# florasion/D-VQVAE

Hardware: AMD Instinct MI355X
Metric: grasps/sec at batch=65536, N=1024 pts, K=512 (higher is better)
Workload: dtype f32 (GEMMs: every fp32 operand as two fp16 pieces, a1 = fp16(a), a2 = fp16((a - a1) * 2^11), weights pre-scaled by one power of two per output row; the 3 partial products a1 b1, a1 b2, a2 b1 are exact in fp32 and accumulate in TWO fp32 accumulators (large / cross terms) on v_mfma_f32_16x16x32_f16; d

## Files before the change

### d-vqvae_amd/csrc/pn_filter.h

```cpp
#pragma once
#include <stddef.h>
#include "pn_slots.h"

constexpr int PN_MAX_TILES = 64;
constexpr int PN_MAX_POINTS = PN_MAX_TILES * PN_TILE_SLOTS;

struct PnGeometry {
    int tiles;
    int deal;
    int Npad;
    long slots;
    size_t h2;
    size_t rec4;
    size_t rec2;
    size_t tstat;
    size_t cbuf;
    bool has_tail() const { return deal < tiles; }
    size_t part() const { return rec4 + rec2; }
    size_t per_sample() const { return h2 + part() + tstat + cbuf; }
};
inline PnGeometry pn_geometry(int N, bool tail_enabled) {
    PnGeometry g;
    g.tiles = (N + PN_TILE_SLOTS - 1) / PN_TILE_SLOTS;
    const int over = N - PN_TILE_SLOTS * (g.tiles - 1);
// ... 12 lines not shown
    auto up = [](size_t n) { return (n + 255) / 256 * 256; };
    const size_t part = up(samples * g.h2), tstat = part + up(samples * g.part()), cbuf = tstat + up(samples * g.tstat);
    return {0, part, part + samples * g.rec4, tstat, cbuf, cbuf + up(samples * g.cbuf)};
}

enum PnAbl : int {
    PN_ABL_NO_H2_STORE = 1,
    PN_ABL_NO_CONV3 = 2,
    PN_ABL_FEW_ROWS = 16,
    PN_ABL_NO_GROUPS = 32,
    PN_ABL_NO_DOTS = 64,
    PN_ABL_NO_CHAIN = 128,
    PN_ABL_NO_PUBLISH = 256,
    PN_ABL_NO_HANDOVER = 512,
    PN_ABL_NO_W3_LOADS = 1024,
    PN_ABL_STAMPS = 4096,
    PN_ABL_CLOCK = 8192,
    PN_ABL_NO_CHUNK_BARRIER = 16384,
    PN_ABL_INJECT_LIE = 32768,
    PN_ABL_INJECT_LOST = 65536,
    PN_ABL_CONSUMER = 131072,
    PN_ABL_SPLIT = 262144,
    PN_ABL_ONE_PER_CU = 524288,
    PN_ABL_VALID = PN_ABL_STAMPS | PN_ABL_CLOCK | PN_ABL_INJECT_LIE | PN_ABL_INJECT_LOST | PN_ABL_ONE_PER_CU
};

struct PnSlot { float *h2, *part, *cbuf; void* part2; unsigned* tstat; };

#ifdef __HIPCC__
#include "dvq_internal.h"

struct PnTrunkWeights {
    const float *w1, *b1, *w2, *b2, *w3, *b3;
    const uint16_t *w2p, *w3p;
    const void* w3f;
    int relu3;
};
inline PnTrunkWeights pn_stn_trunk(const dvq_pointnet_weights* w) {
    return {w->s_w1, w->s_b1, w->s_w2, w->s_b2, w->s_w3, w->s_b3, w->s_w2p, w->s_w3p, w->s_w3f, 1};
}
inline PnTrunkWeights pn_main_trunk(const dvq_pointnet_weights* w) {
    return {w->w1, w->b1, w->w2, w->b2, w->w3, w->b3, w->w2p, w->w3p, w->w3f, 0};
}
struct PnBatch { const float *pc, *trans; int C, N; long B; };

int dvq_launch_pn_trunk(const PnBatch& in, const PnTrunkWeights& w, float* partial, hipStream_t st);
int dvq_launch_pn_filter_front(const PnBatch& in, const PnTrunkWeights& w, const PnSlot& sl, unsigned long long* stats, hipStream_t st);
int dvq_launch_pn_filter_back(const PnBatch& in, const PnTrunkWeights& w, const PnSlot& sl, float* feat, long ld_feat,
// ... 6 lines not shown
```

### d-vqvae_amd/csrc/pointnet.hip

```cpp
#include "dvq_internal.h"
#include "pn_filter.h"
#include <map>
#include <utility>
#include <vector>

namespace {

__global__ void pn_layer1_kernel(const float* __restrict__ pc, int C, int N, int Npad, long B,
                                 const float* __restrict__ trans , const float* __restrict__ W ,
                                 const float* __restrict__ bias, float* __restrict__ out ) {
    const long gid = (long)blockIdx.x * blockDim.x + threadIdx.x;
    const long pt = gid >> 4;
    const int q = (int)(gid & 15);
    if (pt >= B * Npad) return;
    const long b = pt / Npad;
    const int n = (int)(pt % Npad);
    f32x4 y = {0.f, 0.f, 0.f, 0.f};
    if (n < N) {
        const float* src = pc + b * (long)C * N;
        float x0 = src[n], x1 = src[N + n], x2 = src[2 * N + n];
        const float x3 = (C > 3) ? src[3 * N + n] : 0.f;
        if (trans) {
            const float* t = trans + b * 9;
            const float n0 = fmaf(x2, t[6], fmaf(x1, t[3], x0 * t[0]));
// ... 33 lines not shown
        const long v = dvq_knobs().pn_chunk;
        if (v > 0 && v < chunk) chunk = v;
        if (v <= 0) {
            if (chunk > 4096) chunk = 4096;
            if (B >= 2048 && chunk > (B + 3) / 4) chunk = (B + 3) / 4;
        }
    }
    if (chunk > B) chunk = B;
    if (chunk < 1) chunk = 1;
    if (B > 0) chunk = (B + ((B + chunk - 1) / chunk) - 1) / ((B + chunk - 1) / chunk);
    s.chunk = chunk;
    const long launches = B > 0 ? (B + chunk - 1) / chunk : 1;
    s.slots = launches >= 2 ? (dvq_knobs().pn_slots > 0 ? dvq_knobs().pn_slots : 2) : 1;
    if (s.slots > 4) s.slots = 4;
    if (s.slots > 2 * launches) s.slots = (int)(2 * launches);
    char* p = (char*)ws;
    auto take = [&](size_t n) { char* q = p; p += dvq_round_up(n, 256); return (float*)q; };
    const PnSetLayout l = pn_set_layout(s.g, (size_t)chunk);
    for (int i = 0; i < s.slots; ++i) {
        char* set = (char*)take(l.bytes);
        s.slot[i] = PnSlot{(float*)(set + l.h2), (float*)(set + l.part), (float*)(set + l.cbuf), set + l.part2, (unsigned*)(set + l.tstat)};
    }
    s.h1 = s.slots >= 2 ? s.slot[1].h2 : take((size_t)chunk * s.g.Npad * 64 * 4);
    s.stats = (unsigned long long*)take(64);
    s.f0 = take((size_t)chunk * 1024 * 4);
    s.f1 = take((size_t)chunk * 512 * 4);
    s.f2 = take((size_t)chunk * 256 * 4);
    s.tr = take((size_t)(B > 0 ? B : 1) * 16 * 4);
    s.bytes = (size_t)(p - (char*)ws);
    return s;
}

int dense(const float* x, int K, const float* w, const uint16_t* wp, const float* b, long M, int N, int relu, float* y, hipStream_t st) {
    GemmParams p = {};
    p.src[0] = GemmSrc{x, w, (long)K, (long)K, K, 0, wp, (long)N * K};
    p.nsrc = 1;
    p.M = M;
    p.N = N;
    p.bias = b;
    p.out = y;
    p.ldo = N;
    p.relu = relu;
    return dvq_launch_gemm(p, EPI_BIAS, st);
}

bool use_filter(const dvq_pointnet_weights* w, int N) {
    const int fm = dvq_knobs().pn_filter;
// ... 385 lines not shown
```

### d-vqvae_amd/csrc/pointnet_filter.hip

```cpp
#include "dvq_internal.h"
#include "pn_filter.h"
#include <vector>

namespace {

typedef __bf16 qbf16x8 __attribute__((ext_vector_type(8)));
typedef _Float16 qf16x8 __attribute__((ext_vector_type(8)));
typedef _Float16 qf16x2 __attribute__((ext_vector_type(2)));
typedef float qf32x2 __attribute__((ext_vector_type(2)));

constexpr float C_ID = 5.0e-5f;
constexpr float DELTA = 1.0e-6f;
constexpr float NEG_BIG = -3.0e38f;

constexpr int F_STAGE2 = 2 * 64 * 128;
constexpr int IMG_OFF_TI = 1024 * 256, IMG_OFF_WN = IMG_OFF_TI + 4096, IMG_OFF_RN = IMG_OFF_WN + 4096;
constexpr int IMG_OFF_W2 = IMG_OFF_RN + 4096, IMG_OFF_K2 = IMG_OFF_W2 + 2 * 128 * 128, IMG_BYTES = IMG_OFF_K2 + 512;
constexpr int F_STAGE3 = 64 * 256;
constexpr int F_OFF_TB = 2 * F_STAGE3;
constexpr int F_SLOT = 4 * 2 * 2 * 2 * 64;
constexpr int F_OFF_W1 = F_OFF_TB + 8 * 4 * 4 * 64 * 4;
constexpr int F_OFF_B1 = F_OFF_W1 + 64 * 4 * 4;
constexpr int F_OFF_B2 = F_OFF_B1 + 64 * 4;
constexpr int F_OFF_K2 = F_OFF_B2 + 128 * 4;
// ... 602 lines not shown
    s = fmaf(w1[0], c[0], s);
    s = fmaf(w1[1], c[1], s);
    s = fmaf(w1[2], c[2], s);
    s = fmaf(w1[3], c[3], s);
    s += q_dpp<0xB1>(s);
    s += q_dpp<0x4E>(s);
    s += q_dpp<0x141>(s);
    s += q_dpp<0x140>(s);
    return s;
}
__device__ __forceinline__ float exact_dot(const f32x4& w0, const f32x4& w1, const float* __restrict__ hrow, int j) {
    return exact_dot_regs(w0, w1, *reinterpret_cast<const f32x4*>(hrow + 4 * j), *reinterpret_cast<const f32x4*>(hrow + 4 * j + 64));
}
__device__ __forceinline__ float max_nan(float a, float b) { return (a != a || b != b) ? __builtin_nanf("") : fmaxf(a, b); }

__device__ __forceinline__ unsigned f2key(float v) {
    const unsigned u = __float_as_uint(v);
    return (u & 0x80000000u) ? ~u : (u | 0x80000000u);
}
__device__ __forceinline__ float key2f(unsigned k) { return __uint_as_float((k & 0x80000000u) ? (k & 0x7fffffffu) : ~k); }

__device__ unsigned long long g_pn_faults[2];

constexpr int PAIR_CAP = 1024;
constexpr int FB_CAP = 512;
constexpr int SORT_CAP = 3072;
__global__ __launch_bounds__(256, 4) void pn_exact_kernel(const f32x4* __restrict__ part, const qf32x2* __restrict__ part2, int tiles, int deal,
                                                       const float* __restrict__ h2buf,
                                                       int N, int Npad, const float* __restrict__ w3, const float* __restrict__ b3,
                                                       const float* __restrict__ wnorm, const float* __restrict__ rnorm,
                                                       const unsigned* __restrict__ tstat, const float* __restrict__ cbuf, int relu, int exhaustive,
                                                       int pair_cap, int fb_cap, float* __restrict__ feat, long ld_feat,
                                                       unsigned long long* __restrict__ stats, int abl_arg) {
    const int abl = DVQ_DIAG_ON ? abl_arg : 0;
    __shared__ unsigned short cand[1024][4];
    __shared__ unsigned char cand_n[1024];
    __shared__ int pair_list[PAIR_CAP];
    __shared__ int fb_list[FB_CAP];
    __shared__ short all_list[1024];
    __shared__ int pair_count, fb_count, all_count;
    __shared__ float fb_part[4][16];
    __shared__ float hm[PN_MAX_TILES], dm[PN_MAX_TILES], rd[PN_MAX_TILES];
    __shared__ unsigned best_k[1024];
    __shared__ int pcnt[1024];
    __shared__ unsigned sorted[SORT_CAP];
    __shared__ int wave_tot[4];
    const int tid = threadIdx.x, g = tid >> 4, j = tid & 15;
    const long b = blockIdx.x;
    float* wcs = reinterpret_cast<float*>(pcnt);
    const f32x4 cen_a = *reinterpret_cast<const f32x4*>(cbuf + b * 128 + 4 * j), cen_b = *reinterpret_cast<const f32x4*>(cbuf + b * 128 + 4 * j + 64);
    if (tid == 0) { pair_count = 0; fb_count = 0; all_count = 0; }
#pragma unroll
    for (int i = 0; i < 4; ++i) pcnt[tid + 256 * i] = 0;
    int nonfinite_point = 0;
    if (tid < tiles) {
        const unsigned* ts = tstat + 4 * (b * tiles + tid);
        hm[tid] = __uint_as_float(ts[0]) * 1.00001f;
        dm[tid] = __uint_as_float(ts[1]) * 1.00001f;
        rd[tid] = __uint_as_float(ts[2]) * 1.00001f;
        nonfinite_point = ts[3] != 0 && !(abl & PN_ABL_STAMPS);
    }
    if (__syncthreads_or(nonfinite_point)) {
        for (int n = tid; n < 1024; n += 256) feat[b * ld_feat + n] = __builtin_nanf("");
        return;
    }
    const float* h2 = h2buf + b * (long)Npad * 128;
    const bool wrap_small = Npad <= 2 * N;
    const f32x4* pt = part + b * (long)tiles * 1024;
    const qf32x2* pt2 = part2 + b * (long)tiles * 1024;
    const bool stamps = DVQ_DIAG_ON && stats && (abl & PN_ABL_STAMPS);
    unsigned long long tp0 = stamps ? __builtin_amdgcn_s_memtime() : 0ull, tp1 = 0, tp2 = 0, tp3 = 0;
    unsigned n_single = 0, n_multi = 0, n_cand = 0, n_wave = 0, n_suspect = 0;
    float lo_0 = 1.f, lo_1 = 1.f, lo_2 = 1.f, lo_3 = 1.f, hi_0 = 0.f, hi_1 = 0.f, hi_2 = 0.f, hi_3 = 0.f;
    f32x4 nf0 = pt[tid], nf1 = pt[min(1, tiles - 1) * 1024 + tid], nf2 = pt[min(2, tiles - 1) * 1024 + tid], nf3 = pt[min(3, tiles - 1) * 1024 + tid];
    qf32x2 ng0 = pt2[tid], ng1 = pt2[min(1, tiles - 1) * 1024 + tid], ng2 = pt2[min(2, tiles - 1) * 1024 + tid], ng3 = pt2[min(3, tiles - 1) * 1024 + tid];
    float nwn = wnorm[tid], nrn = rnorm[tid];
#pragma unroll 1
    for (int ci = 0; ci < 4; ++ci) {
        const int n = tid + 256 * ci;
        best_k[n] = f2key(NEG_BIG);
        const float wn = nwn, rn = nrn;
        const f32x4 f0 = nf0, f1 = nf1, f2 = nf2, f3 = nf3;
        const qf32x2 g0 = ng0, g1 = ng1, g2 = ng2, g3 = ng3;
        if (ci < 3) {
            const int nx = n + 256;
            nf0 = pt[nx]; nf1 = pt[min(1, tiles - 1) * 1024 + nx]; nf2 = pt[min(2, tiles - 1) * 1024 + nx]; nf3 = pt[min(3, tiles - 1) * 1024 + nx];
            ng0 = pt2[nx]; ng1 = pt2[min(1, tiles - 1) * 1024 + nx]; ng2 = pt2[min(2, tiles - 1) * 1024 + nx]; ng3 = pt2[min(3, tiles - 1) * 1024 + nx];
            nwn = wnorm[nx]; nrn = rnorm[nx];
        }
        float lb, e_all;
        auto bound = [&](int t) { return fmaf(rn, dm[t], fmaf(wn, rd[t], fmaf(C_ID * wn, dm[t], 2.0f * DELTA * wn * hm[t]))); };
        bool nonfinite = false;
        float ub;
        auto fold = [&](float e, float top) {
            nonfinite = nonfinite || !(e < 3.0e38f) || !(fabsf(top) < 3.0e38f);
            e_all = fmaxf(e_all, e);
            lb = fmaxf(lb, top - e);
            ub = fmaxf(ub, top + e);
        };
        {
            const float e0 = bound(0);
            e_all = e0;
            lb = f0[0] - e0;
            ub = f0[0] + e0;
            nonfinite = !(e0 < 3.0e38f) || !(fabsf(f0[0]) < 3.0e38f);
            if (tiles > 1) fold(bound(1), f1[0]);
            if (tiles > 2) fold(bound(2), f2[0]);
            if (tiles > 3) fold(bound(3), f3[0]);
        }
        for (int t0 = 4; t0 < tiles; t0 += 4) {
            float top[4];
#pragma unroll
            for (int u = 0; u < 4; ++u) top[u] = pt[min(t0 + u, tiles - 1) * 1024 + n][0];
#pragma unroll
            for (int u = 0; u < 4; ++u)
                if (t0 + u < tiles) fold(bound(t0 + u), top[u]);
        }
        int cands = 0;
        bool whole = false;
        const bool all = exhaustive || nonfinite || !(e_all < 3.0e38f) || !(lb > NEG_BIG) || !(lb < 3.0e38f);
        if (all) {
            all_list[atomicAdd(&all_count, 1)] = (short)n;
            cand_n[n] = 0;
            continue;
        }
        float lo_c = lb, hi_c = ub;
        auto consider = [&](int t, const f32x4& q, const qf32x2& q45) {
            const float et = bound(t);
            const unsigned suspect = (__float_as_uint(q[3]) >> 16) & 1u;
            n_suspect += suspect;
            if (!suspect && !(q[0] + et >= lb)) return;
            unsigned flags = __float_as_uint(q[3]) & 0xFFFFu;
            auto take = [&](float v) {
                int p = point_of_slot(t, slot_of_id(__float_as_uint(v) & 255u), deal);
                if (p >= N) p = wrap_small ? p - N : p % N;
                if (abl & PN_ABL_FEW_ROWS) p &= 63;
                if (cands < 4) cand[n][cands] = (unsigned short)p;
                else {
                    const int slot = atomicAdd(&pair_count, 1);
                    if (slot < pair_cap) pair_list[slot] = n | (p << 10);
                    else {
                        const unsigned id = __float_as_uint(v);
                        flags |= 1u << pn_group_of_id(id);
                    }
                }
                ++cands;
            };
            const float sc5[5] = {q[0], q[1], q[2], q45[0], q45[1]};
#pragma unroll 1
            for (int k = 0; k < 5; ++k) {
                const float v = k == 0 ? sc5[0] : k == 1 ? sc5[1] : k == 2 ? sc5[2] : k == 3 ? sc5[3] : sc5[4];
                if (!(v + et >= lb)) break;
                take(v);
            }
            while (flags) {
                const int wh = __ffs(flags) - 1;
                flags &= flags - 1;
                const int slot = atomicAdd(&fb_count, 1);
                if (slot < fb_cap) fb_list[slot] = n | (t << 10) | (wh << 20);
                else if (!whole) {
                    whole = true;
                    all_list[atomicAdd(&all_count, 1)] = (short)n;
                }
                ++n_wave;
            }
        };
        f32x4 q0 = f0, q1 = f1, q2 = f2, q3 = f3;
        qf32x2 h0 = g0, h1 = g1, h2q = g2, h3 = g3;
#pragma unroll 1
        for (int t0 = 0; t0 < tiles; t0 += 4) {
            if (t0 > 0) {
                q0 = pt[min(t0, tiles - 1) * 1024 + n]; q1 = pt[min(t0 + 1, tiles - 1) * 1024 + n];
                q2 = pt[min(t0 + 2, tiles - 1) * 1024 + n]; q3 = pt[min(t0 + 3, tiles - 1) * 1024 + n];
                h0 = pt2[min(t0, tiles - 1) * 1024 + n]; h1 = pt2[min(t0 + 1, tiles - 1) * 1024 + n];
                h2q = pt2[min(t0 + 2, tiles - 1) * 1024 + n]; h3 = pt2[min(t0 + 3, tiles - 1) * 1024 + n];
            }
#pragma unroll 1
            for (int u = 0; u < 4 && t0 + u < tiles; ++u) {
                const f32x4 q = u == 0 ? q0 : u == 1 ? q1 : u == 2 ? q2 : q3;
                const qf32x2 q45 = u == 0 ? h0 : u == 1 ? h1 : u == 2 ? h2q : h3;
                consider(t0 + u, q, q45);
            }
        }
        cand_n[n] = whole ? 0 : (unsigned char)min(cands, 4);
        if (whole) { lo_c = 1.f; hi_c = 0.f; }
        lo_0 = ci == 0 ? lo_c : lo_0; hi_0 = ci == 0 ? hi_c : hi_0;
        lo_1 = ci == 1 ? lo_c : lo_1; hi_1 = ci == 1 ? hi_c : hi_1;
        lo_2 = ci == 2 ? lo_c : lo_2; hi_2 = ci == 2 ? hi_c : hi_2;
        lo_3 = ci == 3 ? lo_c : lo_3; hi_3 = ci == 3 ? hi_c : hi_3;
        n_single += cands == 1;
        n_multi += cands != 1;
        n_cand += cands;
    }
    dvq_lds_barrier();
    if (stamps) tp1 = __builtin_amdgcn_s_memtime();
    const int npairs = min(pair_count, pair_cap);
    for (int n = tid; n < 1024; n += 256)
        for (int k = 0; k < cand_n[n]; ++k) atomicAdd(&pcnt[cand[n][k] & 1023], 1);
    for (int i = tid; i < npairs; i += 256) atomicAdd(&pcnt[(pair_list[i] >> 10) & 1023], 1);
    dvq_lds_barrier();
    int total;
    {
        const int c0 = pcnt[4 * tid], c1 = pcnt[4 * tid + 1], c2 = pcnt[4 * tid + 2], c3 = pcnt[4 * tid + 3];
        int incl = c0 + c1 + c2 + c3;
#pragma unroll
        for (int o = 1; o < 64; o <<= 1) {
            const int v = __shfl_up(incl, o);
            if ((tid & 63) >= o) incl += v;
        }
        if ((tid & 63) == 63) wave_tot[tid >> 6] = incl;
        dvq_lds_barrier();
        int base = 0;
        for (int w = 0; w < (tid >> 6); ++w) base += wave_tot[w];
        total = wave_tot[0] + wave_tot[1] + wave_tot[2] + wave_tot[3];
        const int excl = base + incl - (c0 + c1 + c2 + c3);
        pcnt[4 * tid] = excl;
        pcnt[4 * tid + 1] = excl + c0;
        pcnt[4 * tid + 2] = excl + c0 + c1;
        pcnt[4 * tid + 3] = excl + c0 + c1 + c2;
    }
    dvq_lds_barrier();
    const bool by_point = total <= SORT_CAP && !(abl & PN_ABL_NO_DOTS);
    if (by_point) {
        for (int n = tid; n < 1024; n += 256)
            for (int k = 0; k < cand_n[n]; ++k) {
                const int p = cand[n][k];
                sorted[atomicAdd(&pcnt[p & 1023], 1)] = (unsigned)n | ((unsigned)p << 10);
            }
        for (int i = tid; i < npairs; i += 256) {
            const int code = pair_list[i];
            sorted[atomicAdd(&pcnt[(code >> 10) & 1023], 1)] = (unsigned)code;
        }
        dvq_lds_barrier();
        if (stamps) tp2 = __builtin_amdgcn_s_memtime();
        const int per = (total + 15) >> 4, i0 = g * per, i1 = min(total, i0 + per);
        for (int i = i0; i < i1; i += 4) {
            f32x4 w0[4], w1[4], ha[4], hb[4];
            int nn[4];
#pragma unroll
            for (int u = 0; u < 4; ++u) {
                const unsigned code = sorted[min(i + u, i1 - 1)];
                nn[u] = (int)(code & 1023u);
                const unsigned woff = (code & 1023u) * 512u + 16u * (unsigned)j, hoff = (code >> 10) * 512u + 16u * (unsigned)j;
                w0[u] = *reinterpret_cast<const f32x4*>(reinterpret_cast<const char*>(w3) + woff);
                w1[u] = *reinterpret_cast<const f32x4*>(reinterpret_cast<const char*>(w3) + woff + 256);
                ha[u] = *reinterpret_cast<const f32x4*>(reinterpret_cast<const char*>(h2) + hoff);
                hb[u] = *reinterpret_cast<const f32x4*>(reinterpret_cast<const char*>(h2) + hoff + 256);
            }
            float v[4], wc[4];
#pragma unroll
            for (int u = 0; u < 4; ++u) {
                v[u] = exact_dot_regs(w0[u], w1[u], ha[u], hb[u]);
                wc[u] = exact_dot_regs(w0[u], w1[u], cen_a, cen_b);
            }
            if (j == 0) {
#pragma unroll
                for (int u = 0; u < 4; ++u)
                    if (i + u < i1) { atomicMax(&best_k[nn[u]], f2key(v[u])); wcs[nn[u]] = wc[u]; }
            }
        }
    }
    for (int n0 = g; n0 < ((abl & PN_ABL_NO_DOTS) || by_point ? 0 : 1024); n0 += 64) {
        f32x4 w0[4], w1[4], ha[4], hb[4];
        int cn[4];
#pragma unroll
        for (int u = 0; u < 4; ++u) {
            const int n = n0 + 16 * u;
            cn[u] = cand_n[n];
            const float* wr = reinterpret_cast<const float*>(reinterpret_cast<const char*>(w3) + ((unsigned)n * 512u + 16u * (unsigned)j));
            w0[u] = *reinterpret_cast<const f32x4*>(wr);
            w1[u] = *reinterpret_cast<const f32x4*>(wr + 64);
            const float* hr = h2 + (long)(cn[u] ? cand[n][0] : 0) * 128 + 4 * j;
            ha[u] = *reinterpret_cast<const f32x4*>(hr);
            hb[u] = *reinterpret_cast<const f32x4*>(hr + 64);
        }
#pragma unroll
        for (int u = 0; u < 4; ++u) {
            const int n = n0 + 16 * u;
            if (cn[u] == 0) continue;
            float best = exact_dot_regs(w0[u], w1[u], ha[u], hb[u]);
            const float wc = exact_dot_regs(w0[u], w1[u], cen_a, cen_b);
            if (j == 0) wcs[n] = wc;
            if (cn[u] > 1) {
                f32x4 xa[3], xb[3];
#pragma unroll
                for (int k = 1; k < 4; ++k)
                    if (k < cn[u]) {
                        const float* hr = h2 + (long)cand[n][k] * 128 + 4 * j;
                        xa[k - 1] = *reinterpret_cast<const f32x4*>(hr);
                        xb[k - 1] = *reinterpret_cast<const f32x4*>(hr + 64);
                    }
#pragma unroll
                for (int k = 1; k < 4; ++k)
                    if (k < cn[u]) best = fmaxf(best, exact_dot_regs(w0[u], w1[u], xa[k - 1], xb[k - 1]));
            }
            if (j == 0) atomicMax(&best_k[n], f2key(best));
        }
    }
    for (int i = g; i < (by_point ? 0 : npairs); i += 16) {
        const int code = pair_list[i];
        const int n = code & 1023;
        const float* wr = reinterpret_cast<const float*>(reinterpret_cast<const char*>(w3) + ((unsigned)n * 512u + 16u * (unsigned)j));
        const float v = exact_dot(*reinterpret_cast<const f32x4*>(wr), *reinterpret_cast<const f32x4*>(wr + 64), h2 + (long)(code >> 10) * 128, j);
        if (j == 0) atomicMax(&best_k[n], f2key(v));
    }
    if (stamps) tp3 = __builtin_amdgcn_s_memtime();
    const int nfb = (abl & PN_ABL_NO_GROUPS) ? 0 : min(fb_count, fb_cap);
    for (int i = tid >> 6; i < nfb; i += 4) {
        const int code = fb_list[i];
        const int n = code & 1023, t = (code >> 10) & 1023, grp = (code >> 20) & 15;
        const float* wr = reinterpret_cast<const float*>(reinterpret_cast<const char*>(w3) + ((unsigned)n * 512u + 16u * (unsigned)j));
        const f32x4 w0 = *reinterpret_cast<const f32x4*>(wr), w1 = *reinterpret_cast<const f32x4*>(wr + 64);
        float best = NEG_BIG;
        {
            f32x4 ha[4], hb[4];
#pragma unroll
            for (int u = 0; u < 4; ++u) {
                int p = point_of_slot(t, pn_group_slot(grp, 4 * (g & 3) + u), deal);
                if (p >= N) p %= N;
                const float* hr = reinterpret_cast<const float*>(reinterpret_cast<const char*>(h2) + ((unsigned)p * 512u + 16u * (unsigned)j));
                ha[u] = *reinterpret_cast<const f32x4*>(hr);
                hb[u] = *reinterpret_cast<const f32x4*>(hr + 64);
            }
#pragma unroll
            for (int u = 0; u < 4; ++u) best = fmaxf(best, exact_dot_regs(w0, w1, ha[u], hb[u]));
        }
        if (j == 0) atomicMax(&best_k[n], f2key(best));
    }
    dvq_lds_barrier();
// ... 36 lines not shown
#pragma unroll
    for (int ci = 0; ci < 4; ++ci) {
        const int n = tid + 256 * ci;
        const float lo_c = ci == 0 ? lo_0 : ci == 1 ? lo_1 : ci == 2 ? lo_2 : lo_3, hi_c = ci == 0 ? hi_0 : ci == 1 ? hi_1 : ci == 2 ? hi_2 : hi_3;
        if (!(lo_c <= hi_c) || (abl & ~PN_ABL_VALID)) continue;
        const float v = key2f(best_k[n]), wc = wcs[n];
        const float x = v - wc, slack = 4.0e-7f * (fabsf(v) + fabsf(wc));
        if (!(x >= lo_c - slack && x <= hi_c + slack)) {
            all_list[atomicAdd(&all_count, 1)] = (short)n;
            ++n_bad;
        }
    }
    dvq_lds_barrier();
    eval_all_list(all_count);
    if (n_suspect) atomicAdd(&g_pn_faults[0], (unsigned long long)n_suspect);
    if (n_bad) atomicAdd(&g_pn_faults[1], (unsigned long long)n_bad);
    for (int n = tid; n < 1024; n += 256) {
        const unsigned k = best_k[n];
        const float v = (k == 0xffffffffu ? __builtin_nanf("") : key2f(k)) + b3[n];
        feat[b * ld_feat + n] = relu ? (v != v ? v : fmaxf(v, 0.f)) : v;
    }
    if (stamps && tid == 0) {
        const unsigned long long t_end = __builtin_amdgcn_s_memtime();
        atomicAdd(stats + 4, tp1 - tp0); atomicAdd(stats + 5, tp2 - tp1); atomicAdd(stats + 6, tp3 - tp2); atomicAdd(stats + 7, t_end - tp3);
    }
    if (stats) {
        if (n_single) atomicAdd(stats + 0, (unsigned long long)n_single);
        if (n_multi) atomicAdd(stats + 1, (unsigned long long)n_multi);
        if (n_wave) atomicAdd(stats + 2, (unsigned long long)n_wave);
        if (n_cand) atomicAdd(stats + 3, (unsigned long long)n_cand);
    }
}

constexpr int CENTER_SPB = 4;
template <int C>
__global__ __launch_bounds__(256) void pn_center_kernel(const float* __restrict__ pc, const float* __restrict__ trans, int N, long B,
                                                        const float* __restrict__ W1, const float* __restrict__ b1,
                                                        const float* __restrict__ W2, const float* __restrict__ b2,
                                                        float* __restrict__ cbuf, unsigned* __restrict__ tstat, int tiles) {
    __shared__ float w2t[64][129];
    __shared__ float h1c[4][64];
    __shared__ float h2c[4][128];
    const int tid = threadIdx.x, q = tid >> 6, k = tid & 63;
    for (int i = tid; i < 128 * 64; i += 256) w2t[i & 63][i >> 6] = W2[i];
    for (int sb = 0; sb < CENTER_SPB; ++sb) {
        const long b = (long)blockIdx.x * CENTER_SPB + sb;
        if (b >= B) break;
        for (int i = tid; i < 4 * tiles; i += 256) tstat[b * 4 * tiles + i] = 0u;
        {
// ... 104 lines not shown
static int pn_abl() { const char* e = getenv("DVQ_PN_ABL"); return e ? atoi(e) : 0; }
#else
static constexpr int pn_abl() { return 0; }
#endif

using TrunkFilterKernel = decltype(&pn_trunk_filter_kernel<3, false>);
static TrunkFilterKernel trunk_filter_kernel(int C, bool tail) {
    static const TrunkFilterKernel k[2][2] = {{&pn_trunk_filter_kernel<3, false>, &pn_trunk_filter_kernel<3, true>},
                                              {&pn_trunk_filter_kernel<4, false>, &pn_trunk_filter_kernel<4, true>}};
    return k[C == 4][tail];
}
static decltype(&pn_center_kernel<3>) center_kernel(int C) { return C == 4 ? &pn_center_kernel<4> : &pn_center_kernel<3>; }

int dvq_launch_pn_filter_front(const PnBatch& in, const PnTrunkWeights& w, const PnSlot& sl, unsigned long long* stats, hipStream_t st) {
    PnGeometry g;
    DVQ_PROPAGATE(filter_geometry(in.N, &g));
    static DvqOncePerDevice attr_once[2][2];
    for (int c = 0; c < 2; ++c)
        for (int tail = 0; tail < 2; ++tail)
            DVQ_PROPAGATE(dvq_lds_limit(attr_once[c][tail], reinterpret_cast<const void*>(trunk_filter_kernel(3 + c, tail)),
                                        tail ? F_LDS_TAIL : (DVQ_DIAG_ON ? 100 * 1024 : F_LDS), "pointnet"));
    const long B = in.B, grid = B * g.deal;
    DVQ_REQUIRE(B * g.tiles < (1L << 31), "pointnet: grid too large");
    if (stats && hipMemsetAsync(stats, 0, 64, st) != hipSuccess) {
        dvq_set_error("pointnet: hipMemsetAsync failed");
        return DVQ_ELAUNCH;
    }
    {
        DVQ_PROF("pn_center", 2.0 * (double)B * 4 * (4.0 * 64 + 64.0 * 128), (double)B * (64 + 512), st);
        DVQ_LAUNCH(center_kernel(in.C), dim3((unsigned)((B + CENTER_SPB - 1) / CENTER_SPB)), dim3(256), 0, st, in.pc, in.trans, in.N, B, w.w1,
                   w.b1, w.w2, w.b2, sl.cbuf, sl.tstat, g.tiles);
    }
    DVQ_CHECK_LAUNCH("pn_center");
    const double pts = (double)B * g.slots;
    const int abl = pn_abl();
    auto launch = [&](bool tail, int lds, hipStream_t s, int abl_arg) {
        DVQ_LAUNCH(trunk_filter_kernel(in.C, tail), dim3((unsigned)(tail ? (B + 3) / 4 : grid)), dim3(256), lds, s, in.pc, in.trans, in.N, g.Npad,
                   g.tiles, g.deal, B, w.w1, w.b1, w.b2, (const char*)w.w3f, sl.h2, (f32x4*)sl.part, (qf32x2*)sl.part2, sl.tstat, sl.cbuf, abl_arg);
    };
    {
        DVQ_PROF("pn_trunk", 2.0 * pts * (4.0 * 64 + 64.0 * 128 + 128.0 * 1024), pts * (16 + 512) + (double)grid * 16384, st);
#ifdef DVQ_DIAG
        if ((abl & PN_ABL_SPLIT) && in.C == 4) {
            static hipStream_t side = nullptr;
            static hipEvent_t ev0 = nullptr, ev1 = nullptr;
            if (!side) { (void)hipStreamCreateWithFlags(&side, hipStreamNonBlocking); (void)hipEventCreateWithFlags(&ev0, hipEventDisableTiming); (void)hipEventCreateWithFlags(&ev1, hipEventDisableTiming); }
            (void)hipEventRecord(ev0, st);
// ... 34 lines not shown
                   reinterpret_cast<const float*>((const char*)w.w3f + IMG_OFF_RN), tstat, sl.cbuf, w.relu3, exhaustive, pair_cap, fb_cap,
                   feat, ld_feat, stats, abl);
    }
    DVQ_CHECK_LAUNCH("pn_exact");
    if (stats && (abl & PN_ABL_STAMPS)) {
        const long nrec = B * tiles;
        std::vector<unsigned> ts((size_t)nrec * 4);
        (void)hipStreamSynchronize(st);
        (void)hipMemcpy(ts.data(), tstat, ts.size() * 4, hipMemcpyDeviceToHost);
        double a = 0, b2_ = 0, c = 0, d = 0;
        for (long i = 0; i < nrec; ++i) {
            const unsigned v = ts[4 * i + 3];
            a += v & 255; b2_ += (v >> 8) & 255; c += (v >> 16) & 255; d += (v >> 24) & 255;
        }
        if (abl & PN_ABL_CLOCK) {
            double mhz = 0;
            for (long i = 0; i < nrec; ++i) mhz += ts[4 * i + 3];
            fprintf(stderr, "[dvq pn] in-kernel clock of the trunk kernel: %.0f MHz (s_memtime over s_memrealtime, mean over %ld workgroups)\n", mhz / nrec, nrec);
        } else
        fprintf(stderr, "[dvq pn] mean phase ticks per workgroup (s_memtime): start->loaded %.0f, conv1+conv2 %.0f, centre/convert %.0f, conv3 loop %.0f\n",
                a / nrec * 64, b2_ / nrec * 64, c / nrec * 64, d / nrec * 512);
    }
    if (stats) {
        unsigned long long h[8] = {0, 0, 0, 0, 0, 0, 0, 0};
        (void)hipStreamSynchronize(st);
        (void)hipMemcpy(h, stats, sizeof h, hipMemcpyDeviceToHost);
        (void)hipMemset((void*)stats, 0, sizeof h);
        const double tot = (double)B * 1024;
        fprintf(stderr, "[dvq pn] B=%ld N=%d: one candidate %.4f, other counts %.4f of the channels, flagged 16-point groups %.5f per channel; %.3f candidate dots per channel\n",
                B, N, h[0] / tot, h[1] / tot, h[2] / tot, h[3] / tot);
        if (abl & PN_ABL_STAMPS)
            fprintf(stderr, "[dvq pn] exact stage, mean cycles per workgroup: records -> candidates %.0f, sort by point %.0f, candidate dots %.0f, flagged groups + checks + store %.0f\n",
                    (double)h[4] / B, (double)h[5] / B, (double)h[6] / B, (double)h[7] / B);
    }
    return DVQ_OK;
}

int dvq_pn_fault_counters(unsigned long long* out2, int reset) {
    if (hipDeviceSynchronize() != hipSuccess || hipMemcpyFromSymbol(out2, HIP_SYMBOL(g_pn_faults), 16) != hipSuccess) {
        dvq_set_error("pointnet_fault_counters: reading the device counters failed");
        return DVQ_ELAUNCH;
    }
    if (reset) {
        const unsigned long long z[2] = {0, 0};
        if (hipMemcpyToSymbol(HIP_SYMBOL(g_pn_faults), z, 16) != hipSuccess) {
            dvq_set_error("pointnet_fault_counters: resetting the device counters failed");
            return DVQ_ELAUNCH;
        }
    }
    return DVQ_OK;
}
```

Baseline: 183,600.

## Add anchor pre-pass with exact dots to tighten candidate pruning in exact stage

The exact max-pool stage now runs a first pass that picks each channel's most likely winning point (anchor), sorts those anchors by point and computes their exact dots up front. The resulting exact value, adjusted by the centre term, raises the lower bound used to prune further candidates (rule 2). A second rule skips flagged 16-point groups whose remaining scores cannot reach the bound (rule 1). The fixed 4-candidate per-channel arrays and the unsorted fallback path are replaced by one sorted pair list with a larger capacity. This trades an extra scan over the tile records and extra barriers for fewer candidate dots and fewer fallback group evaluations.

```diff
diff --git a/d-vqvae_amd/csrc/pn_filter.h b/d-vqvae_amd/csrc/pn_filter.h
--- a/d-vqvae_amd/csrc/pn_filter.h
+++ b/d-vqvae_amd/csrc/pn_filter.h
@@ -58,8 +58,12 @@
     PN_ABL_CONSUMER = 131072,
     PN_ABL_SPLIT = 262144,
     PN_ABL_ONE_PER_CU = 524288,
-    PN_ABL_VALID = PN_ABL_STAMPS | PN_ABL_CLOCK | PN_ABL_INJECT_LIE | PN_ABL_INJECT_LOST | PN_ABL_ONE_PER_CU
+    PN_ABL_NO_RULE1 = 1048576,
+    PN_ABL_NO_RULE2 = 2097152,
+    PN_ABL_VALID = PN_ABL_STAMPS | PN_ABL_CLOCK | PN_ABL_INJECT_LIE | PN_ABL_INJECT_LOST | PN_ABL_ONE_PER_CU | PN_ABL_NO_RULE1 | PN_ABL_NO_RULE2
 };
+
+constexpr size_t PN_STATS_BYTES = 128;
 
 struct PnSlot { float *h2, *part, *cbuf; void* part2; unsigned* tstat; };
 
diff --git a/d-vqvae_amd/csrc/pointnet.hip b/d-vqvae_amd/csrc/pointnet.hip
--- a/d-vqvae_amd/csrc/pointnet.hip
+++ b/d-vqvae_amd/csrc/pointnet.hip
@@ -79,7 +79,7 @@
         s.slot[i] = PnSlot{(float*)(set + l.h2), (float*)(set + l.part), (float*)(set + l.cbuf), set + l.part2, (unsigned*)(set + l.tstat)};
     }
     s.h1 = s.slots >= 2 ? s.slot[1].h2 : take((size_t)chunk * s.g.Npad * 64 * 4);
-    s.stats = (unsigned long long*)take(64);
+    s.stats = (unsigned long long*)take(PN_STATS_BYTES);
     s.f0 = take((size_t)chunk * 1024 * 4);
     s.f1 = take((size_t)chunk * 512 * 4);
     s.f2 = take((size_t)chunk * 256 * 4);
diff --git a/d-vqvae_amd/csrc/pointnet_filter.hip b/d-vqvae_amd/csrc/pointnet_filter.hip
--- a/d-vqvae_amd/csrc/pointnet_filter.hip
+++ b/d-vqvae_amd/csrc/pointnet_filter.hip
@@ -648,9 +648,9 @@
 
 __device__ unsigned long long g_pn_faults[2];
 
-constexpr int PAIR_CAP = 1024;
+constexpr int PAIR_CAP = 2048;
 constexpr int FB_CAP = 512;
-constexpr int SORT_CAP = 3072;
+constexpr unsigned short NO_ANCHOR = 0xFFFFu;
 __global__ __launch_bounds__(256, 4) void pn_exact_kernel(const f32x4* __restrict__ part, const qf32x2* __restrict__ part2, int tiles, int deal,
                                                        const float* __restrict__ h2buf,
                                                        int N, int Npad, const float* __restrict__ w3, const float* __restrict__ b3,
@@ -659,8 +659,7 @@
                                                        int pair_cap, int fb_cap, float* __restrict__ feat, long ld_feat,
                                                        unsigned long long* __restrict__ stats, int abl_arg) {
     const int abl = DVQ_DIAG_ON ? abl_arg : 0;
-    __shared__ unsigned short cand[1024][4];
-    __shared__ unsigned char cand_n[1024];
+    __shared__ unsigned short anchor[1024];
     __shared__ int pair_list[PAIR_CAP];
     __shared__ int fb_list[FB_CAP];
     __shared__ short all_list[1024];
@@ -668,14 +667,17 @@
     __shared__ float fb_part[4][16];
     __shared__ float hm[PN_MAX_TILES], dm[PN_MAX_TILES], rd[PN_MAX_TILES];
     __shared__ unsigned best_k[1024];
+    __shared__ float wcs[1024];
     __shared__ int pcnt[1024];
-    __shared__ unsigned sorted[SORT_CAP];
+    __shared__ unsigned sorted[PAIR_CAP];
     __shared__ int wave_tot[4];
+    __shared__ unsigned row_mask[32];
+    static_assert(PAIR_CAP >= 1024, "sorted[] holds the 1 024 anchors");
     const int tid = threadIdx.x, g = tid >> 4, j = tid & 15;
     const long b = blockIdx.x;
-    float* wcs = reinterpret_cast<float*>(pcnt);
     const f32x4 cen_a = *reinterpret_cast<const f32x4*>(cbuf + b * 128 + 4 * j), cen_b = *reinterpret_cast<const f32x4*>(cbuf + b * 128 + 4 * j + 64);
     if (tid == 0) { pair_count = 0; fb_count = 0; all_count = 0; }
+    if (tid < 32) row_mask[tid] = 0;
 #pragma unroll
     for (int i = 0; i < 4; ++i) pcnt[tid + 256 * i] = 0;
     int nonfinite_point = 0;
@@ -695,8 +697,151 @@
     const f32x4* pt = part + b * (long)tiles * 1024;
     const qf32x2* pt2 = part2 + b * (long)tiles * 1024;
     const bool stamps = DVQ_DIAG_ON && stats && (abl & PN_ABL_STAMPS);
-    unsigned long long tp0 = stamps ? __builtin_amdgcn_s_memtime() : 0ull, tp1 = 0, tp2 = 0, tp3 = 0;
-    unsigned n_single = 0, n_multi = 0, n_cand = 0, n_wave = 0, n_suspect = 0;
+    unsigned long long tp[8] = {0, 0, 0, 0, 0, 0, 0, 0};
+    if (stamps) tp[0] = __builtin_amdgcn_s_memtime();
+    unsigned n_single = 0, n_multi = 0, n_cand = 0, n_wave = 0, n_suspect = 0, n_rows = 0;
+    auto bound_of = [&](float wn, float rn, int t) { return fmaf(rn, dm[t], fmaf(wn, rd[t], fmaf(C_ID * wn, dm[t], 2.0f * DELTA * wn * hm[t]))); };
+    struct Scan { float lb, ub, e_all, top_star; int t_star; bool all; };
+    auto scan_tiles = [&](int n, float wn, float rn, float top0, float top1, float top2, float top3) {
+        Scan s;
+        bool nonfinite = false;
+        auto fold = [&](int t, float top) {
+            const float e = bound_of(wn, rn, t), l = top - e;
+            nonfinite = nonfinite || !(e < 3.0e38f) || !(fabsf(top) < 3.0e38f);
+            s.e_all = fmaxf(s.e_all, e);
+            if (l > s.lb) { s.t_star = t; s.top_star = top; }
+            s.lb = fmaxf(s.lb, l);
+            s.ub = fmaxf(s.ub, top + e);
+        };
+        {
+            const float e0 = bound_of(wn, rn, 0);
+            s.e_all = e0;
+            s.lb = top0 - e0;
+            s.ub = top0 + e0;
+            s.t_star = 0;
+            s.top_star = top0;
+            nonfinite = !(e0 < 3.0e38f) || !(fabsf(top0) < 3.0e38f);
+            if (tiles > 1) fold(1, top1);
+            if (tiles > 2) fold(2, top2);
+            if (tiles > 3) fold(3, top3);
+        }
+        for (int t0 = 4; t0 < tiles; t0 += 4) {
+            float top[4];
+#pragma unroll
+            for (int u = 0; u < 4; ++u) top[u] = pt[min(t0 + u, tiles - 1) * 1024 + n][0];
+#pragma unroll
+            for (int u = 0; u < 4; ++u)
+                if (t0 + u < tiles) fold(t0 + u, top[u]);
+        }
+        s.all = exhaustive || nonfinite || !(s.e_all < 3.0e38f) || !(s.lb > NEG_BIG) || !(s.lb < 3.0e38f);
+        return s;
+    };
+    auto point_of_score = [&](int t, float v) {
+        int p = point_of_slot(t, slot_of_id(__float_as_uint(v) & 255u), deal);
+        if (p >= N) p = wrap_small ? p - N : p % N;
+        if (abl & PN_ABL_FEW_ROWS) p &= 63;
+        return p;
+    };
+    auto sort_by_point = [&](auto code_at, int count, bool first) {
+        for (int i = tid; i < count; i += 256) {
+            const unsigned code = code_at(i);
+            if (code != ~0u) atomicAdd(&pcnt[(code >> 10) & 1023], 1);
+        }
+        dvq_lds_barrier();
+        const int c0 = pcnt[4 * tid], c1 = pcnt[4 * tid + 1], c2 = pcnt[4 * tid + 2], c3 = pcnt[4 * tid + 3];
+        if (stats) {
+            const unsigned m = (unsigned)(c0 != 0) | (unsigned)(c1 != 0) << 1 | (unsigned)(c2 != 0) << 2 | (unsigned)(c3 != 0) << 3;
+            const int sh = 4 * (tid & 7);
+            if (first) { if (m) atomicOr(&row_mask[tid >> 3], m << sh); n_rows += __popc(m); }
+            else n_rows += __popc(m & ~(row_mask[tid >> 3] >> sh));
+        }
+        int incl = c0 + c1 + c2 + c3;
+#pragma unroll
+        for (int o = 1; o < 64; o <<= 1) {
+            const int v = __shfl_up(incl, o);
+            if ((tid & 63) >= o) incl += v;
+        }
+        if ((tid & 63) == 63) wave_tot[tid >> 6] = incl;
+        dvq_lds_barrier();
+        int base = 0;
+        for (int w = 0; w < (tid >> 6); ++w) base += wave_tot[w];
+        const int total = wave_tot[0] + wave_tot[1] + wave_tot[2] + wave_tot[3];
+        const int excl = base + incl - (c0 + c1 + c2 + c3);
+        pcnt[4 * tid] = excl;
+        pcnt[4 * tid + 1] = excl + c0;
+        pcnt[4 * tid + 2] = excl + c0 + c1;
+        pcnt[4 * tid + 3] = excl + c0 + c1 + c2;
+        dvq_lds_barrier();
+        for (int i = tid; i < count; i += 256) {
+            const unsigned code = code_at(i);
+            if (code != ~0u) sorted[atomicAdd(&pcnt[(code >> 10) & 1023], 1)] = code;
+        }
+        dvq_lds_barrier();
+        return total;
+    };
+    auto dots = [&](int total, bool first) {
+        const int per = (total + 15) >> 4, i0 = g * per, i1 = min(total, i0 + per);
+        for (int i = i0; i < i1; i += 4) {
+            f32x4 w0[4], w1[4], ha[4], hb[4];
+            int nn[4];
+#pragma unroll
+            for (int u = 0; u < 4; ++u) {
+                const unsigned code = sorted[min(i + u, i1 - 1)];
+                nn[u] = (int)(code & 1023u);
+                const unsigned woff = (code & 1023u) * 512u + 16u * (unsigned)j, hoff = (code >> 10) * 512u + 16u * (unsigned)j;
+                w0[u] = *reinterpret_cast<const f32x4*>(reinterpret_cast<const char*>(w3) + woff);
+                w1[u] = *reinterpret_cast<const f32x4*>(reinterpret_cast<const char*>(w3) + woff + 256);
+                ha[u] = *reinterpret_cast<const f32x4*>(reinterpret_cast<const char*>(h2) + hoff);
+                hb[u] = *reinterpret_cast<const f32x4*>(reinterpret_cast<const char*>(h2) + hoff + 256);
+            }
+            float v[4], wc[4];
+#pragma unroll
+            for (int u = 0; u < 4; ++u) {
+                v[u] = exact_dot_regs(w0[u], w1[u], ha[u], hb[u]);
+                wc[u] = first ? exact_dot_regs(w0[u], w1[u], cen_a, cen_b) : 0.f;
+            }
+            if (j == 0) {
+#pragma unroll
+                for (int u = 0; u < 4; ++u)
+                    if (i + u < i1) {
+                        if (first) { best_k[nn[u]] = f2key(v[u]); wcs[nn[u]] = wc[u]; }
+                        else atomicMax(&best_k[nn[u]], f2key(v[u]));
+                    }
+            }
+        }
+    };
+    {
+        float top[4][4], wn[4], rn[4];
+#pragma unroll
+        for (int ci = 0; ci < 4; ++ci) {
+            const int n = tid + 256 * ci;
+#pragma unroll
+            for (int u = 0; u < 4; ++u) top[ci][u] = pt[min(u, tiles - 1) * 1024 + n][0];
+            wn[ci] = wnorm[n]; rn[ci] = rnorm[n];
+        }
+#pragma unroll
+        for (int ci = 0; ci < 4; ++ci) {
+            const int n = tid + 256 * ci;
+            const Scan s = scan_tiles(n, wn[ci], rn[ci], top[ci][0], top[ci][1], top[ci][2], top[ci][3]);
+            best_k[n] = f2key(NEG_BIG);
+            wcs[n] = 0.f;
+            if (s.all) {
+                all_list[atomicAdd(&all_count, 1)] = (short)n;
+                anchor[n] = NO_ANCHOR;
+            } else
+                anchor[n] = (unsigned short)point_of_score(s.t_star, s.top_star);
+        }
+    }
+    dvq_lds_barrier();
+    if (stamps) tp[1] = __builtin_amdgcn_s_memtime();
+    auto anchor_code = [&](int n) { const unsigned p = anchor[n]; return p == NO_ANCHOR ? ~0u : (unsigned)n | (p << 10); };
+    const int n_anchor = sort_by_point(anchor_code, 1024, true);
+#pragma unroll
+    for (int i = 0; i < 4; ++i) pcnt[tid + 256 * i] = 0;
+    if (stamps) tp[2] = __builtin_amdgcn_s_memtime();
+    if (!(abl & PN_ABL_NO_DOTS)) dots(n_anchor, true);
+    dvq_lds_barrier();
+    if (stamps) tp[3] = __builtin_amdgcn_s_memtime();
     float lo_0 = 1.f, lo_1 = 1.f, lo_2 = 1.f, lo_3 = 1.f, hi_0 = 0.f, hi_1 = 0.f, hi_2 = 0.f, hi_3 = 0.f;
     f32x4 nf0 = pt[tid], nf1 = pt[min(1, tiles - 1) * 1024 + tid], nf2 = pt[min(2, tiles - 1) * 1024 + tid], nf3 = pt[min(3, tiles - 1) * 1024 + tid];
     qf32x2 ng0 = pt2[tid], ng1 = pt2[min(1, tiles - 1) * 1024 + tid], ng2 = pt2[min(2, tiles - 1) * 1024 + tid], ng3 = pt2[min(3, tiles - 1) * 1024 + tid];
@@ -704,7 +849,6 @@
 #pragma unroll 1
     for (int ci = 0; ci < 4; ++ci) {
         const int n = tid + 256 * ci;
-        best_k[n] = f2key(NEG_BIG);
         const float wn = nwn, rn = nrn;
         const f32x4 f0 = nf0, f1 = nf1, f2 = nf2, f3 = nf3;
         const qf32x2 g0 = ng0, g1 = ng1, g2 = ng2, g3 = ng3;
@@ -714,74 +858,52 @@
             ng0 = pt2[nx]; ng1 = pt2[min(1, tiles - 1) * 1024 + nx]; ng2 = pt2[min(2, tiles - 1) * 1024 + nx]; ng3 = pt2[min(3, tiles - 1) * 1024 + nx];
             nwn = wnorm[nx]; nrn = rnorm[nx];
         }
-        float lb, e_all;
-        auto bound = [&](int t) { return fmaf(rn, dm[t], fmaf(wn, rd[t], fmaf(C_ID * wn, dm[t], 2.0f * DELTA * wn * hm[t]))); };
-        bool nonfinite = false;
-        float ub;
-        auto fold = [&](float e, float top) {
-            nonfinite = nonfinite || !(e < 3.0e38f) || !(fabsf(top) < 3.0e38f);
-            e_all = fmaxf(e_all, e);
-            lb = fmaxf(lb, top - e);
-            ub = fmaxf(ub, top + e);
-        };
-        {
-            const float e0 = bound(0);
-            e_all = e0;
-            lb = f0[0] - e0;
-            ub = f0[0] + e0;
-            nonfinite = !(e0 < 3.0e38f) || !(fabsf(f0[0]) < 3.0e38f);
-            if (tiles > 1) fold(bound(1), f1[0]);
-            if (tiles > 2) fold(bound(2), f2[0]);
-            if (tiles > 3) fold(bound(3), f3[0]);
-        }
-        for (int t0 = 4; t0 < tiles; t0 += 4) {
-            float top[4];
-#pragma unroll
-            for (int u = 0; u < 4; ++u) top[u] = pt[min(t0 + u, tiles - 1) * 1024 + n][0];
-#pragma unroll
-            for (int u = 0; u < 4; ++u)
-                if (t0 + u < tiles) fold(bound(t0 + u), top[u]);
-        }
-        int cands = 0;
+        const Scan s = scan_tiles(n, wn, rn, f0[0], f1[0], f2[0], f3[0]);
+        if (s.all) continue;
+        const float lb = s.lb;
+        float L = lb;
+        if (!(abl & PN_ABL_NO_RULE2)) {
+            const float v1 = key2f(best_k[n]), wc1 = wcs[n];
+            L = fmaxf(lb, (v1 - wc1) - 4.0e-7f * (fabsf(v1) + fabsf(wc1)));
+        }
+        int cands = 1;
         bool whole = false;
-        const bool all = exhaustive || nonfinite || !(e_all < 3.0e38f) || !(lb > NEG_BIG) || !(lb < 3.0e38f);
-        if (all) {
-            all_list[atomicAdd(&all_count, 1)] = (short)n;
-            cand_n[n] = 0;
-            continue;
-        }
-        float lo_c = lb, hi_c = ub;
+        float lo_c = lb, hi_c = s.ub;
         auto consider = [&](int t, const f32x4& q, const qf32x2& q45) {
-            const float et = bound(t);
+            const float et = bound_of(wn, rn, t);
             const unsigned suspect = (__float_as_uint(q[3]) >> 16) & 1u;
             n_suspect += suspect;
-            if (!suspect && !(q[0] + et >= lb)) return;
+            if (!suspect && !(q[0] + et >= L)) return;
             unsigned flags = __float_as_uint(q[3]) & 0xFFFFu;
+            unsigned forced = suspect ? 0xFFFFu : 0u;
             auto take = [&](float v) {
-                int p = point_of_slot(t, slot_of_id(__float_as_uint(v) & 255u), deal);
-                if (p >= N) p = wrap_small ? p - N : p % N;
-                if (abl & PN_ABL_FEW_ROWS) p &= 63;
-                if (cands < 4) cand[n][cands] = (unsigned short)p;
+                const int p = point_of_score(t, v);
+                const int slot = atomicAdd(&pair_count, 1);
+                if (slot < pair_cap) pair_list[slot] = n | (p << 10);
                 else {
-                    const int slot = atomicAdd(&pair_count, 1);
-                    if (slot < pair_cap) pair_list[slot] = n | (p << 10);
-                    else {
-                        const unsigned id = __float_as_uint(v);
-                        flags |= 1u << pn_group_of_id(id);
-                    }
+                    const unsigned bit = 1u << pn_group_of_id(__float_as_uint(v));
+                    flags |= bit;
+                    forced |= bit;
                 }
                 ++cands;
             };
             const float sc5[5] = {q[0], q[1], q[2], q45[0], q45[1]};
 #pragma unroll 1
-            for (int k = 0; k < 5; ++k) {
+            for (int k = (t == s.t_star ? 1 : 0); k < 5; ++k) {
                 const float v = k == 0 ? sc5[0] : k == 1 ? sc5[1] : k == 2 ? sc5[2] : k == 3 ? sc5[3] : sc5[4];
-                if (!(v + et >= lb)) break;
+                if (!(v + et >= L)) break;
                 take(v);
             }
             while (flags) {
                 const int wh = __ffs(flags) - 1;
                 flags &= flags - 1;
+                if (!((forced >> wh) & 1u) && !(abl & PN_ABL_NO_RULE1)) {
+                    auto of_group = [&](float v) { return pn_group_of_id(__float_as_uint(v)) == wh; };
+                    const bool m0 = of_group(sc5[0]), m1 = of_group(sc5[1]), m2 = of_group(sc5[2]), m3 = of_group(sc5[3]), m4 = of_group(sc5[4]);
+                    const float second = m4 ? sc5[4] : m3 ? sc5[3] : m2 ? sc5[2] : m1 ? sc5[1] : sc5[0];
+                    const float u = (int)m0 + (int)m1 + (int)m2 + (int)m3 + (int)m4 >= 2 ? second : sc5[4];
+                    if (u + et < L) continue;
+                }
                 const int slot = atomicAdd(&fb_count, 1);
                 if (slot < fb_cap) fb_list[slot] = n | (t << 10) | (wh << 20);
                 else if (!whole) {
@@ -808,7 +930,6 @@
                 consider(t0 + u, q, q45);
             }
         }
-        cand_n[n] = whole ? 0 : (unsigned char)min(cands, 4);
         if (whole) { lo_c = 1.f; hi_c = 0.f; }
         lo_0 = ci == 0 ? lo_c : lo_0; hi_0 = ci == 0 ? hi_c : hi_0;
         lo_1 = ci == 1 ? lo_c : lo_1; hi_1 = ci == 1 ? hi_c : hi_1;
@@ -819,118 +940,12 @@
         n_cand += cands;
     }
     dvq_lds_barrier();
-    if (stamps) tp1 = __builtin_amdgcn_s_memtime();
+    if (stamps) tp[4] = __builtin_amdgcn_s_memtime();
     const int npairs = min(pair_count, pair_cap);
-    for (int n = tid; n < 1024; n += 256)
-        for (int k = 0; k < cand_n[n]; ++k) atomicAdd(&pcnt[cand[n][k] & 1023], 1);
-    for (int i = tid; i < npairs; i += 256) atomicAdd(&pcnt[(pair_list[i] >> 10) & 1023], 1);
-    dvq_lds_barrier();
-    int total;
-    {
-        const int c0 = pcnt[4 * tid], c1 = pcnt[4 * tid + 1], c2 = pcnt[4 * tid + 2], c3 = pcnt[4 * tid + 3];
-        int incl = c0 + c1 + c2 + c3;
-#pragma unroll
-        for (int o = 1; o < 64; o <<= 1) {
-            const int v = __shfl_up(incl, o);
-            if ((tid & 63) >= o) incl += v;
-        }
-        if ((tid & 63) == 63) wave_tot[tid >> 6] = incl;
-        dvq_lds_barrier();
-        int base = 0;
-        for (int w = 0; w < (tid >> 6); ++w) base += wave_tot[w];
-        total = wave_tot[0] + wave_tot[1] + wave_tot[2] + wave_tot[3];
-        const int excl = base + incl - (c0 + c1 + c2 + c3);
-        pcnt[4 * tid] = excl;
-        pcnt[4 * tid + 1] = excl + c0;
-        pcnt[4 * tid + 2] = excl + c0 + c1;
-        pcnt[4 * tid + 3] = excl + c0 + c1 + c2;
-    }
-    dvq_lds_barrier();
-    const bool by_point = total <= SORT_CAP && !(abl & PN_ABL_NO_DOTS);
-    if (by_point) {
-        for (int n = tid; n < 1024; n += 256)
-            for (int k = 0; k < cand_n[n]; ++k) {
-                const int p = cand[n][k];
-                sorted[atomicAdd(&pcnt[p & 1023], 1)] = (unsigned)n | ((unsigned)p << 10);
-            }
-        for (int i = tid; i < npairs; i += 256) {
-            const int code = pair_list[i];
-            sorted[atomicAdd(&pcnt[(code >> 10) & 1023], 1)] = (unsigned)code;
-        }
-        dvq_lds_barrier();
-        if (stamps) tp2 = __builtin_amdgcn_s_memtime();
-        const int per = (total + 15) >> 4, i0 = g * per, i1 = min(total, i0 + per);
-        for (int i = i0; i < i1; i += 4) {
-            f32x4 w0[4], w1[4], ha[4], hb[4];
-            int nn[4];
-#pragma unroll
-            for (int u = 0; u < 4; ++u) {
-                const unsigned code = sorted[min(i + u, i1 - 1)];
-                nn[u] = (int)(code & 1023u);
-                const unsigned woff = (code & 1023u) * 512u + 16u * (unsigned)j, hoff = (code >> 10) * 512u + 16u * (unsigned)j;
-                w0[u] = *reinterpret_cast<const f32x4*>(reinterpret_cast<const char*>(w3) + woff);
-                w1[u] = *reinterpret_cast<const f32x4*>(reinterpret_cast<const char*>(w3) + woff + 256);
-                ha[u] = *reinterpret_cast<const f32x4*>(reinterpret_cast<const char*>(h2) + hoff);
-                hb[u] = *reinterpret_cast<const f32x4*>(reinterpret_cast<const char*>(h2) + hoff + 256);
-            }
-            float v[4], wc[4];
-#pragma unroll
-            for (int u = 0; u < 4; ++u) {
-                v[u] = exact_dot_regs(w0[u], w1[u], ha[u], hb[u]);
-                wc[u] = exact_dot_regs(w0[u], w1[u], cen_a, cen_b);
-            }
-            if (j == 0) {
-#pragma unroll
-                for (int u = 0; u < 4; ++u)
-                    if (i + u < i1) { atomicMax(&best_k[nn[u]], f2key(v[u])); wcs[nn[u]] = wc[u]; }
-            }
-        }
-    }
-    for (int n0 = g; n0 < ((abl & PN_ABL_NO_DOTS) || by_point ? 0 : 1024); n0 += 64) {
-        f32x4 w0[4], w1[4], ha[4], hb[4];
-        int cn[4];
-#pragma unroll
-        for (int u = 0; u < 4; ++u) {
-            const int n = n0 + 16 * u;
-            cn[u] = cand_n[n];
-            const float* wr = reinterpret_cast<const float*>(reinterpret_cast<const char*>(w3) + ((unsigned)n * 512u + 16u * (unsigned)j));
-            w0[u] = *reinterpret_cast<const f32x4*>(wr);
-            w1[u] = *reinterpret_cast<const f32x4*>(wr + 64);
-            const float* hr = h2 + (long)(cn[u] ? cand[n][0] : 0) * 128 + 4 * j;
-            ha[u] = *reinterpret_cast<const f32x4*>(hr);
-            hb[u] = *reinterpret_cast<const f32x4*>(hr + 64);
-        }
-#pragma unroll
-        for (int u = 0; u < 4; ++u) {
-            const int n = n0 + 16 * u;
-            if (cn[u] == 0) continue;
-            float best = exact_dot_regs(w0[u], w1[u], ha[u], hb[u]);
-            const float wc = exact_dot_regs(w0[u], w1[u], cen_a, cen_b);
-            if (j == 0) wcs[n] = wc;
-            if (cn[u] > 1) {
-                f32x4 xa[3], xb[3];
-#pragma unroll
-                for (int k = 1; k < 4; ++k)
-                    if (k < cn[u]) {
-                        const float* hr = h2 + (long)cand[n][k] * 128 + 4 * j;
-                        xa[k - 1] = *reinterpret_cast<const f32x4*>(hr);
-                        xb[k - 1] = *reinterpret_cast<const f32x4*>(hr + 64);
-                    }
-#pragma unroll
-                for (int k = 1; k < 4; ++k)
-                    if (k < cn[u]) best = fmaxf(best, exact_dot_regs(w0[u], w1[u], xa[k - 1], xb[k - 1]));
-            }
-            if (j == 0) atomicMax(&best_k[n], f2key(best));
-        }
-    }
-    for (int i = g; i < (by_point ? 0 : npairs); i += 16) {
-        const int code = pair_list[i];
-        const int n = code & 1023;
-        const float* wr = reinterpret_cast<const float*>(reinterpret_cast<const char*>(w3) + ((unsigned)n * 512u + 16u * (unsigned)j));
-        const float v = exact_dot(*reinterpret_cast<const f32x4*>(wr), *reinterpret_cast<const f32x4*>(wr + 64), h2 + (long)(code >> 10) * 128, j);
-        if (j == 0) atomicMax(&best_k[n], f2key(v));
-    }
-    if (stamps) tp3 = __builtin_amdgcn_s_memtime();
+    const int n_sorted = sort_by_point([&](int i) { return (unsigned)pair_list[i]; }, npairs, false);
+    if (stamps) tp[5] = __builtin_amdgcn_s_memtime();
+    if (!(abl & PN_ABL_NO_DOTS)) dots(n_sorted, false);
+    if (stamps) tp[6] = __builtin_amdgcn_s_memtime();
     const int nfb = (abl & PN_ABL_NO_GROUPS) ? 0 : min(fb_count, fb_cap);
     for (int i = tid >> 6; i < nfb; i += 4) {
         const int code = fb_list[i];
@@ -1013,9 +1028,12 @@
     }
     if (stamps && tid == 0) {
         const unsigned long long t_end = __builtin_amdgcn_s_memtime();
-        atomicAdd(stats + 4, tp1 - tp0); atomicAdd(stats + 5, tp2 - tp1); atomicAdd(stats + 6, tp3 - tp2); atomicAdd(stats + 7, t_end - tp3);
+        atomicAdd(stats + 4, (tp[1] - tp[0]) + (tp[4] - tp[3])); atomicAdd(stats + 5, (tp[2] - tp[1]) + (tp[5] - tp[4]));
+        atomicAdd(stats + 6, (tp[3] - tp[2]) + (tp[6] - tp[5])); atomicAdd(stats + 7, t_end - tp[6]);
+        atomicAdd(stats + 9, tp[3] - tp[0]);
     }
     if (stats) {
+        if (n_rows) atomicAdd(stats + 8, (unsigned long long)n_rows);
         if (n_single) atomicAdd(stats + 0, (unsigned long long)n_single);
         if (n_multi) atomicAdd(stats + 1, (unsigned long long)n_multi);
         if (n_wave) atomicAdd(stats + 2, (unsigned long long)n_wave);
@@ -1166,7 +1184,7 @@
                                         tail ? F_LDS_TAIL : (DVQ_DIAG_ON ? 100 * 1024 : F_LDS), "pointnet"));
     const long B = in.B, grid = B * g.deal;
     DVQ_REQUIRE(B * g.tiles < (1L << 31), "pointnet: grid too large");
-    if (stats && hipMemsetAsync(stats, 0, 64, st) != hipSuccess) {
+    if (stats && hipMemsetAsync(stats, 0, PN_STATS_BYTES, st) != hipSuccess) {
         dvq_set_error("pointnet: hipMemsetAsync failed");
         return DVQ_ELAUNCH;
     }
@@ -1247,16 +1265,18 @@
                 a / nrec * 64, b2_ / nrec * 64, c / nrec * 64, d / nrec * 512);
     }
     if (stats) {
-        unsigned long long h[8] = {0, 0, 0, 0, 0, 0, 0, 0};
+        unsigned long long h[PN_STATS_BYTES / 8] = {};
         (void)hipStreamSynchronize(st);
         (void)hipMemcpy(h, stats, sizeof h, hipMemcpyDeviceToHost);
         (void)hipMemset((void*)stats, 0, sizeof h);
         const double tot = (double)B * 1024;
         fprintf(stderr, "[dvq pn] B=%ld N=%d: one candidate %.4f, other counts %.4f of the channels, flagged 16-point groups %.5f per channel; %.3f candidate dots per channel\n",
                 B, N, h[0] / tot, h[1] / tot, h[2] / tot, h[3] / tot);
+        fprintf(stderr, "[dvq pn] B=%ld N=%d: distinct conv2 rows fetched per cloud <= %.1f (%.1f candidate points + 16 per flagged group)\n",
+                B, N, (double)(h[8] + 16 * h[2]) / B, (double)h[8] / B);
         if (abl & PN_ABL_STAMPS)
-            fprintf(stderr, "[dvq pn] exact stage, mean cycles per workgroup: records -> candidates %.0f, sort by point %.0f, candidate dots %.0f, flagged groups + checks + store %.0f\n",
-                    (double)h[4] / B, (double)h[5] / B, (double)h[6] / B, (double)h[7] / B);
+            fprintf(stderr, "[dvq pn] exact stage, mean cycles per workgroup: records -> candidates %.0f, sort by point %.0f, candidate dots %.0f, flagged groups + checks + store %.0f; of these the anchor pass %.0f\n",
+                    (double)h[4] / B, (double)h[5] / B, (double)h[6] / B, (double)h[7] / B, (double)h[9] / B);
     }
     return DVQ_OK;
 }
```

Measured after the change: 188,200, median of 6. 2.5% higher.
